# MarbleHE/ABC

Hardware: AMD Instinct MI355X
Metric: homomorphic mul+relin/sec, CKKS N=2^14 (higher is better)
Workload: dtype u64 (transforms: exact integer arithmetic in f64); 1 GPU; CKKS N=16384, 4 data limbs {50,40,40,40} + special 50-bit prime, ct x ct multiply + relinearize; total_batch=8192, batch_rank0=8192

## Files before the change

### abc_amd/csrc/abc_context.hip

```cpp
#include <cstdlib>
#include <cstring>
#include <mutex>

#include "../../include/abc_hip.h"
#include <dlfcn.h>

#include "abc_context.hpp"
#include "abc_host_math.hpp"
#include "abc_sample.hpp"

namespace abc {

static thread_local std::string g_err;
void set_error(const std::string &msg) { g_err = msg; }

static bool env_on(const char *name) {
  const char *e = std::getenv(name);
  return e && !(e[0] == '0' && e[1] == 0);
}
void read_switches(abc_hip_ctx *c) {
  abc_hip_ctx::Switches s;
  s.no_fused = env_on("ABC_HIP_NO_FUSED");
  s.no_split = env_on("ABC_HIP_NO_SPLIT");
  s.no_split4 = env_on("ABC_HIP_NO_SPLIT4");
  s.no_isplit = env_on("ABC_HIP_NO_ISPLIT");
  s.no_gsplit = env_on("ABC_HIP_NO_GSPLIT");
  s.no_bsplit = env_on("ABC_HIP_NO_BSPLIT");
  s.no_mixed = env_on("ABC_HIP_NO_MIXED");
  s.no_pack = env_on("ABC_HIP_NO_PACK");
  s.no_key_twin = env_on("ABC_HIP_NO_KEY_TWIN");
  s.no_bmul = env_on("ABC_HIP_NO_BMUL");
  s.no_iks = env_on("ABC_HIP_NO_IKS");
  s.no_lean_front = env_on("ABC_HIP_NO_LEAN_FRONT");
  s.no_tensor_intt = env_on("ABC_HIP_NO_TENSOR_INTT");
  s.no_galois_fusion = env_on("ABC_HIP_NO_GALOIS_FUSION");
  s.main_two_per_cu = env_on("ABC_HIP_MAIN_TWO_PER_CU");
  s.host_sampling = env_on("ABC_HIP_HOST_SAMPLING");
  if (const char *e = std::getenv("ABC_HIP_CHUNK")) s.chunk = (size_t)std::atol(e);
  if (const char *e = std::getenv("ABC_HIP_FEW_LIMBS")) s.few_limbs = (size_t)std::atol(e);
  if (const char *e = std::getenv("ABC_HIP_LEAN_LIMIT")) s.lean_limit = (size_t)std::atol(e);
  if (const char *e = std::getenv("ABC_HIP_PASS0_TARGET_LIMIT")) s.pass0_target_limit = (size_t)std::atol(e);
  if (const char *e = std::getenv("ABC_HIP_BFV_SCRATCH_MB")) s.bfv_scratch_mb = (size_t)std::atol(e);
  if (const char *e = std::getenv("ABC_HIP_LANES")) {
    s.lanes = std::atoi(e);
    if (s.lanes < 1) s.lanes = 1;
    if (s.lanes > abc_hip_ctx::kMaxLanes) s.lanes = abc_hip_ctx::kMaxLanes;
  }
  c->sw = s;
  RouteFacts &f = c->facts;
  f = RouteFacts{};
  f.scheme = c->scheme; f.logn = c->logn; f.K = c->K; f.L = c->L; f.nB = c->nB;
  f.use_fp = c->use_fp; f.behz_fp = c->behz_fp;
  f.big_block_log = big_block_log();
  for (int j = 0; j < c->K; j++) f.bits[j] = (unsigned char)c->h_mods[j].bits;
  f.sw = s;
  f.finish();
}

static Mod make_mod(uint64_t q, int logn, bool ntt) {
  using namespace host;
  Mod m{};
  m.q = q;
  m.two_q = 2 * q;
  const int k = bitlen(q);
  m.bits = (u32)k;
  m.shift = (u32)(k - 1);
  m.mu = (uint64_t)((((u128)1) << (k + 63)) / q);
  m.qd = (double)q;
  m.qinv = 1.0 / (double)q;
  if (ntt) {
    const uint64_t n = 1ull << logn;
    m.inv_n = invmod(n % q, q);
    m.inv_n_s = shoup(m.inv_n, q);
    if (fp_ok(m.bits)) {
      m.inv_n_c = m.inv_n > q / 2 ? -(double)(q - m.inv_n) : (double)m.inv_n;
      m.inv_n_cq = m.inv_n_c / m.qd;
    }
  }
  return m;
}

static void fill_twiddles(uint64_t q, int logn, uint64_t *dst ) {
  using namespace host;
  const size_t n = (size_t)1 << logn;
  const uint64_t psi = min_primitive_root(2 * n, q);
  uint64_t *fwd = dst, *inv = dst + 2 * n;
  uint64_t p = 1;
  for (size_t i = 0; i < n; i++) {
    fwd[2 * (size_t)bitrev((uint32_t)i, logn)] = p;
    p = mulmod(p, psi, q);
  }
  const uint64_t ipsi = invmod(psi, q);
  p = 1;
  for (size_t i = 0; i < n; i++) {
    inv[2 * (size_t)bitrev((uint32_t)i, logn)] = p;
    p = mulmod(p, ipsi, q);
  }
  for (size_t i = 0; i < n; i++) {
    fwd[2 * i + 1] = shoup(fwd[2 * i], q);
    inv[2 * i + 1] = shoup(inv[2 * i], q);
  }
}

static void fill_fp_twiddles(uint64_t q, size_t n, const uint64_t *src , double *dst ) {
  for (size_t i = 0; i < 2 * n; i++) {
    const uint64_t w = src[2 * i];
    dst[i] = w > q / 2 ? -(double)(q - w) : (double)w;
  }
}

static int build_context(abc_hip_ctx *c) {
  using namespace host;
  const int logn = c->logn, K = c->K, L = c->L;
  const size_t N = (size_t)c->n;
  const bool bfv = (c->scheme == ABC_HIP_SCHEME_BFV);
  std::vector<uint64_t> qs(c->primes.begin(), c->primes.begin() + L);
  const uint64_t qsp = c->primes[K - 1];
  DevConst &k = c->h_cst;
  std::memset(&k, 0, sizeof(k));

  c->mod_values.assign(c->primes.begin(), c->primes.end());
  std::vector<uint64_t> Bp;
  uint64_t m_sk = 0, gamma = 0;
  if (bfv) {
    bool fp_aux = !env_on("ABC_HIP_NO_FP64") && !env_on("ABC_HIP_BEHZ_SEAL_BASE");
    for (uint64_t q : c->primes) fp_aux = fp_aux && fp_ok((u32)bitlen(q));
    const int aux_bits = fp_aux ? 50 : 61;
    int nB = L;
    if (32 + bitlen(c->t) + prod_bitlen(qs) >= aux_bits * L + aux_bits) nB++;
    gamma = ntt_primes(N, 61, 2)[1];
    if (!fp_aux) {
      auto aux = ntt_primes(N, 61, (size_t)nB + 2);
      m_sk = aux[0];
      Bp.assign(aux.begin() + 2, aux.end());
    } else {
      std::vector<uint64_t> alt;
      for (uint64_t p : ntt_primes(N, 50, (size_t)nB + 1 + (size_t)K)) {
        bool clash = false;
        for (uint64_t q : c->primes) clash = clash || (p == q);
        if (!clash && alt.size() < (size_t)nB + 1) alt.push_back(p);
      }
      if (alt.size() < (size_t)nB + 1) throw std::runtime_error("not enough 50-bit NTT primes for the BEHZ auxiliary base");
      m_sk = alt[0];
      Bp.assign(alt.begin() + 1, alt.end());
    }
    c->behz_fp = fp_aux && L <= 10 && !env_on("ABC_HIP_BEHZ_INT_KERNELS");
    c->nB = nB;
    c->nBsk = nB + 1;
    for (uint64_t b : Bp) c->mod_values.push_back(b);
    c->mod_values.push_back(m_sk);
    c->mod_values.push_back(gamma);
    c->mod_values.push_back(c->t);
  }
  const int nmods = (int)c->mod_values.size();
  const int id_bsk = K, id_gamma = K + c->nBsk, id_t = K + c->nBsk + 1;
  c->h_mods.clear();
  std::vector<uint64_t> h_tw((size_t)nmods * 4 * N, 0);
  std::vector<double> h_ftw((size_t)nmods * 2 * N, 0.0);
  for (int i = 0; i < nmods; i++) {
    const bool ntt = !(bfv && i == id_gamma);
    c->h_mods.push_back(make_mod(c->mod_values[i], logn, ntt));
    if (ntt) fill_twiddles(c->mod_values[i], logn, h_tw.data() + (size_t)i * 4 * N);
    if (ntt && fp_ok(c->h_mods.back().bits))
      fill_fp_twiddles(c->mod_values[i], N, h_tw.data() + (size_t)i * 4 * N, h_ftw.data() + (size_t)i * 2 * N);
  }

  for (int j = 0; j < L; j++) {
    const uint64_t q = qs[j];
    k.inv_special[j] = invmod(qsp % q, q);
    k.inv_special_s[j] = shoup(k.inv_special[j], q);
    k.special_mod_q[j] = qsp % q;
    k.special_mod_q_s[j] = shoup(k.special_mod_q[j], q);
    k.inv_special_c[j] = k.inv_special[j] > q / 2 ? -(double)(q - k.inv_special[j]) : (double)k.inv_special[j];
    k.inv_special_cq[j] = k.inv_special_c[j] / (double)q;
    k.special_c[j] = k.special_mod_q[j] > q / 2 ? -(double)(q - k.special_mod_q[j]) : (double)k.special_mod_q[j];
    k.special_cq[j] = k.special_c[j] / (double)q;
  }
  for (int l = 1; l < L; l++)
    for (int j = 0; j < l; j++) {
      k.inv_qlast[l][j] = invmod(qs[l] % qs[j], qs[j]);
      k.inv_qlast_s[l][j] = shoup(k.inv_qlast[l][j], qs[j]);
      k.inv_qlast_c[l][j] = k.inv_qlast[l][j] > qs[j] / 2 ? -(double)(qs[j] - k.inv_qlast[l][j]) : (double)k.inv_qlast[l][j];
      k.inv_qlast_cq[l][j] = k.inv_qlast_c[l][j] / (double)qs[j];
    }

  std::vector<uint32_t> slot_map;
  if (bfv) {
    const uint64_t t = c->t;
    k.t = t;
// ... 767 lines not shown
```

### abc_amd/csrc/abc_kernels_fused.hip

```cpp
#include <type_traits>

#include "abc_context.hpp"
#include "abc_host_math.hpp"

namespace abc {

template <int LB>
__global__ __launch_bounds__((1 << LB) / 16) void k_fused_tensor_intt(DevCtx c, const u64 *__restrict__ a,
                                                                      const u64 *__restrict__ b, u64 *__restrict__ c01,
                                                                      u64 *__restrict__ c2coef, u64 *__restrict__ c2ntt, int nl) {
  __shared__ u64 lds[lds_words(LB)];
  const int j = blockIdx.x % nl;
  const size_t ct = blockIdx.x / nl;
  const size_t N = (size_t)1 << LB, pw = (size_t)nl * N;
  const Mod m = c.mods[j];
  const NttTable t = ntt_table(c, j);
  const u64 *__restrict__ a0 = a + ct * 2 * pw + j * N, *__restrict__ a1 = a0 + pw;
  const u64 *__restrict__ b0 = b + ct * 2 * pw + j * N, *__restrict__ b1 = b0 + pw;
  u64 *__restrict__ o0 = c01 + ct * 2 * pw + j * N, *__restrict__ o1 = o0 + pw;
  u64 *__restrict__ dcoef = c2coef + (ct * nl + j) * N, *__restrict__ dntt = c2ntt + (ct * nl + j) * N;
  ntt_inv_block<LB>(
      lds,
      [&](int, int i) {
        const u64 x0 = a0[i], x1 = a1[i], y0 = b0[i], y1 = b1[i];
// ... 348 lines not shown
    ntt_inv_block_a<LB, FpArith>(
        lds, ld,
        [&](int, int i, double v) {
          const double d = fp_mul_lazy(v, m.inv_n_c, m.inv_n_cq, m.qd) - (fp_from_u64(src[i]) + fix);
          o[i] = fp_to_canon(fp_mul_lazy(d, inv, inv_q, m.qd), m.qd, m.qinv);
        },
        t, m, 0, 0);
  }
}

template <int LB>
__global__ __launch_bounds__((1 << LB) / 16) void k_fused_tensor_decomp_fp(DevCtx c, const u64 *__restrict__ a,
                                                                           const u64 *__restrict__ b, u64 *__restrict__ c01,
                                                                           u64 *__restrict__ c2ntt, u64 *__restrict__ dec, int nl) {
  __shared__ double lds[lds_words(LB)];
  const int j = blockIdx.x % nl;
  const size_t ct = blockIdx.x / nl;
  const size_t N = (size_t)1 << LB;
  double src[16];
  {
    const Mod m = mod_at(c, j);
    const FpTable t = fp_table(c, j);
    TensorFront front(a, b, c01, c2ntt, ct, j, nl, N, m);
    ntt_inv_block_a<LB, FpArith>(
        lds, [&](int r, int i) { return front(r, i); },
        [&](int r, int, double v) {
          const double w = fp_centre(fp_mul_lazy(v, m.inv_n_c, m.inv_n_cq, m.qd), m.qd, m.qinv);
          src[r] = w < 0.0 ? w + m.qd : w;
        },
        t, m, 0, 0);
  }
  for (int I = 0; I <= nl; I++) {
    if (I == j) continue;
    const int ki = (I == nl) ? c.K - 1 : I;
    const Mod m = mod_at(c, ki);
    const FpTable t = fp_table(c, ki);
    u64 *__restrict__ dst = dec + ((ct * (nl + 1) + I) * nl + j) * N;
    block_sync_lds();
    ntt_fwd_block_a<LB, FpArith>(
        lds, [&](int r, int) { return src[r]; }, [&](int, int i, double v) { dst[i] = fp_to_lazy(v, m.qd, m.qinv); }, t, m, 0, 0);
  }
}

template <int LB>
__device__ __forceinline__ void store_half_done(double *__restrict__ dst, double (&y)[16], int p, const FpK &kk, int kind) {
  constexpr size_t N = (size_t)1 << LB;
  constexpr int SH = LB - 4;
  if (kind == 0) {
#pragma unroll
    for (int k = 0; k < 16; k++) dst[(k << SH) + p] = y[k];
  } else if (kind == 1) {
#pragma unroll
    for (int k = 0; k < 16; k++) pack_store<1>(dst, N, (size_t)(k << SH) + p, fp_centre(y[k], kk.q, kk.qinv));
  } else {
#pragma unroll
    for (int k = 0; k < 16; k++) pack_store<2>(dst, N, (size_t)(k << SH) + p, fp_centre(y[k], kk.q, kk.qinv));
  }
}


template <int LB, bool CKKS, bool GAL>
__global__ __launch_bounds__((1 << LB) / 16) void k_fused_operand_pass0_fp(DevCtx c, const u64 *__restrict__ src, size_t src_stride,
                                                                           double *__restrict__ part, int nl, int per_target,
                                                                           u32 gelt, int padded) {
  static_assert(LB == 14, "split transforms are laid out for N = 2^14");
  __shared__ double lds[CKKS ? lds_words(LB) : 1];
  const size_t N = (size_t)1 << LB;
  const unsigned wg = per_target ? blockIdx.x / (unsigned)(nl + 1) : blockIdx.x;
  const int only = per_target ? (int)(blockIdx.x % (unsigned)(nl + 1)) : -1;
  const int j = wg % nl;
  const size_t ct = wg / nl;
  const int tid = threadIdx.x;
  const u64 *__restrict__ sp = src + ct * src_stride + (size_t)j * N;
  double x[16];
  if constexpr (CKKS) {
    const Mod m = mod_at(c, j);
    const FpTable t = fp_table(c, j);
    ntt_inv_block_a<LB, FpArith>(
        lds, [&](int, int i) { return fp_from_u64(sp[galois_ntt_src<GAL>((u32)i, gelt, LB)]); },
        [&](int r, int, double v) {
          double w = fp_centre(fp_mul_lazy(v, m.inv_n_c, m.inv_n_cq, m.qd), m.qd, m.qinv);
          x[r] = w < 0.0 ? w + m.qd : w;
        },
        t, m, 0, 0);
  } else if (gelt) {
    const u64 qj = c.mods[j].q;
#pragma unroll
    for (int k = 0; k < 16; k++) {
      bool neg;
      const u64 v = sp[galois_coef_src((u32)((k << 10) + tid), gelt, LB, neg)];
      x[k] = fp_from_u64(neg ? neg_mod(v, qj) : v);
    }
  } else {
#pragma unroll
    for (int k = 0; k < 16; k++) x[k] = fp_from_u64(sp[(k << 10) + tid]);
  }
  const int hi0[1] = {0};
  for (int I = 0; I <= nl; I++) {
    if (CKKS && I == j) continue;
    if (only >= 0 && I != only) continue;
    const int ki = (I == nl) ? c.K - 1 : I;
    const Mod m = mod_at(c, ki);
    const FpTable t = fp_table(c, ki);
    const FpK kk = FpArith::consts(m);
    double y[16];
#pragma unroll
    for (int k = 0; k < 16; k++) y[k] = x[k];
    fwd_pass<FpArith, LB, 0, 4>(y, hi0, t, kk, 0, 0);
    double *__restrict__ dst = part + ((ct * (nl + 1) + I) * nl + j) * ((padded & 1) ? (size_t)c.ps : N);
    store_half_done<LB>(dst, y, tid, kk, ((padded & 2) && I < nl) ? pack_kind(m.bits) : 0);
  }
}

template <int LB>
__global__ __launch_bounds__((1 << LB) / 16) void k_split2_tensor_pass0_fp(DevCtx c, const u64 *__restrict__ a,
                                                                           const u64 *__restrict__ b, double *__restrict__ part,
                                                                           int nl, int pack) {
  static_assert(LB == 14, "split transforms are laid out for N = 2^14");
  __shared__ double lds[lds_words(LB)];
  const int j = blockIdx.x % nl;
  const size_t ct = blockIdx.x / nl;
  const size_t N = (size_t)1 << LB, pw = (size_t)nl * N;
  double src[16];
  {
    const Mod m = mod_at(c, j);
    const FpTable t = fp_table(c, j);
    const u64 *__restrict__ a1 = a + ct * 2 * pw + pw + (size_t)j * N, *__restrict__ b1 = b + ct * 2 * pw + pw + (size_t)j * N;
    const double q = m.qd, qinv = m.qinv;
    ntt_inv_block_a<LB, FpArith>(
        lds, [&](int, int i) { return fp_mulmod(fp_from_u64(a1[i]), fp_from_u64(b1[i]), q, qinv); },
        [&](int r, int, double v) {
          const double w = fp_centre(fp_mul_lazy(v, m.inv_n_c, m.inv_n_cq, m.qd), m.qd, m.qinv);
          src[r] = w < 0.0 ? w + m.qd : w;
        },
        t, m, 0, 0);
  }
  const int tid = threadIdx.x;
  const int hi0[1] = {0};
  for (int I = 0; I <= nl; I++) {
    if (I == j) continue;
    const int ki = (I == nl) ? c.K - 1 : I;
    const Mod m = mod_at(c, ki);
    const FpTable t = fp_table(c, ki);
    const FpK kk = FpArith::consts(m);
    double y[16];
#pragma unroll
    for (int k = 0; k < 16; k++) y[k] = src[k];
    fwd_pass<FpArith, LB, 0, 4>(y, hi0, t, kk, 0, 0);
    double *__restrict__ dst = part + ((ct * (nl + 1) + I) * nl + j) * (size_t)c.ps;
    store_half_done<LB>(dst, y, tid, kk, (pack && I < nl) ? pack_kind(m.bits) : 0);
  }
}

template <int NL>
__global__ __launch_bounds__(NL ? NL * 64 : 768) void k_split_special_fp(DevCtx c, const double *__restrict__ part, const u64 *__restrict__ key,
                                                                         const double *__restrict__ keyf, double *__restrict__ tsp_half,
                                                                         int nl_rt) {
  extern __shared__ double dyn[];
  const int nl = NL ? NL : nl_rt;
  const int J = __builtin_amdgcn_readfirstlane((int)(threadIdx.x >> 6));
  const int lane = threadIdx.x & 63;
  const int blk = blockIdx.x & 15;
  const size_t ct = (size_t)(blockIdx.x >> 4);
  const size_t N = (size_t)c.n, base = (size_t)blk << 10;
  const int ki = c.K - 1;
  const Mod m = mod_at(c, ki);
  const FpTable t = fp_table(c, ki);
  const double q = m.qd, qinv = m.qinv;
  {
    double *buf = dyn + J * lds_words(10);
    const double *__restrict__ src = part + ((ct * (nl + 1) + nl) * nl + J) * (size_t)c.ps + base;
    ntt_fwd_block_a<10, FpTail>(
        buf, [&](int, int i) { return fp_centre(src[i], q, qinv); }, [&](int, int i, double v) { buf[lds_pad(i)] = v; }, t, m, 4, blk,
        lane);
  }
  __syncthreads();
  for (int e = 2 * (int)threadIdx.x; e < 1024; e += 2 * (int)blockDim.x) {
    double s0[2] = {0.0, 0.0}, s1[2] = {0.0, 0.0};
#pragma unroll
    for (int Jx = 0; Jx < (NL ? NL : 12); Jx++) {
      if (!NL && Jx >= nl) break;
      const f64x2 v = *reinterpret_cast<const f64x2 *>(dyn + Jx * lds_words(10) + lds_pad(e));
      const size_t i0 = (((size_t)Jx * 2 + 0) * c.K + ki) * N + base + e, i1 = i0 + (size_t)c.K * N;
      f64x2 k0, k1;
      if (keyf) {
        k0 = *reinterpret_cast<const f64x2 *>(keyf + i0);
        k1 = *reinterpret_cast<const f64x2 *>(keyf + i1);
      } else {
        const u64x2 r0 = *reinterpret_cast<const u64x2 *>(key + i0), r1 = *reinterpret_cast<const u64x2 *>(key + i1);
        k0.x = fp_from_u64(r0.x); k0.y = fp_from_u64(r0.y);
        k1.x = fp_from_u64(r1.x); k1.y = fp_from_u64(r1.y);
      }
      s0[0] += fp_mulmod(v.x, k0.x, q, qinv);
      s0[1] += fp_mulmod(v.y, k0.y, q, qinv);
      s1[0] += fp_mulmod(v.x, k1.x, q, qinv);
      s1[1] += fp_mulmod(v.y, k1.y, q, qinv);
      if (Jx == 7) {
#pragma unroll
        for (int k = 0; k < 2; k++) {
          s0[k] = fp_centre(s0[k], q, qinv);
          s1[k] = fp_centre(s1[k], q, qinv);
        }
      }
    }
    f64x2 r;
    r.x = fp_centre(s0[0], q, qinv); r.y = fp_centre(s0[1], q, qinv);
    *reinterpret_cast<f64x2 *>(dyn + lds_pad(e)) = r;
    r.x = fp_centre(s1[0], q, qinv); r.y = fp_centre(s1[1], q, qinv);
    *reinterpret_cast<f64x2 *>(dyn + lds_words(10) + lds_pad(e)) = r;
  }
  __syncthreads();
  for (int comp = J; comp < 2; comp += nl) {
    double *buf = dyn + comp * lds_words(10);
    double *__restrict__ dst = tsp_half + (ct * 2 + comp) * (size_t)c.ps + base;
    ntt_inv_block_a<10, FpArith>(
        buf, [&](int, int i) { return buf[lds_pad(i)]; }, [&](int, int i, double v) { dst[i] = v; }, t, m, 4, blk, lane);
  }
}

static void launch_split_special(hipStream_t st, abc_hip_ctx *c, size_t cc, int nl, const double *part, const u64 *key, double *tsp_half) {
  const dim3 grid((unsigned)(cc * 16)), block(64 * nl);
  const size_t lds = (size_t)((nl < 2 ? 2 : nl) * lds_words(10)) * 8;
  const double *keyf = key_twin_lookup(c, key);
#define ABC_SP(NLV) hipLaunchKernelGGL((k_split_special_fp<NLV>), grid, block, lds, st, c->dc, part, key, keyf, tsp_half, nl)
  switch (nl) {
    case 1: ABC_SP(1); break;
    case 2: ABC_SP(2); break;
    case 3: ABC_SP(3); break;
    case 4: ABC_SP(4); break;
    default: ABC_SP(0); break;
  }
#undef ABC_SP
}

struct FusedScratch {
  u64 *coef, *ntt, *dec, *ksacc, *tsp, *tlast, *c01;
};
static inline FusedScratch carve(u64 *base, size_t chunk, int nl, size_t N) {
  FusedScratch s;
  s.coef = base;
  s.ntt = s.coef + chunk * nl * N;
  s.dec = s.ntt + chunk * nl * N;
  s.ksacc = s.dec + chunk * nl * (nl + 1) * N;
  s.tsp = s.ksacc + chunk * 2 * nl * N;
  s.tlast = s.tsp + chunk * 2 * N;
  s.c01 = s.tlast + chunk * 2 * N;
  return s;
}


template <int LB>
__global__ __launch_bounds__(256) void k_split3_pass_fp(DevCtx c, const double *__restrict__ tsp_half, double *__restrict__ tpart, int nl,
                                                        int pack) {
  static_assert(LB == 14, "split transforms are laid out for N = 2^14");
  const size_t cc = blockIdx.x >> 2;
  const int p = (int)((blockIdx.x & 3) << 8) + (int)threadIdx.x;
  const int hi0[1] = {0};
  double x[16];
  {
    const Mod ms = mod_at(c, c.K - 1);
    const FpTable ts = fp_table(c, c.K - 1);
    const FpK ks = FpArith::consts(ms);
    const double *__restrict__ src = tsp_half + cc * (size_t)c.ps;
#pragma unroll
    for (int k = 0; k < 16; k++) x[k] = src[(k << 10) + p];
    FpArith::centre16(x, ks);
    inv_pass<FpArith, LB, 0, 4>(x, hi0, ts, ks, 0, 0);
    const double half = (double)(ms.q >> 1);
#pragma unroll
    for (int k = 0; k < 16; k++) {
      const double w = fp_centre(fp_mul_lazy(x[k], ms.inv_n_c, ms.inv_n_cq, ms.qd) + half, ms.qd, ms.qinv);
      x[k] = w < 0.0 ? w + ms.qd : w;
    }
  }
  const u64 half = c.mods[c.K - 1].q >> 1;
  for (int j = 0; j < nl; j++) {
    const Mod m = mod_at(c, j);
    const FpTable t = fp_table(c, j);
    const FpK kk = FpArith::consts(m);
    const u64 hm = reduce64(half, m);
    const double fix = hm ? (double)(m.q - hm) : 0.0;
    double y[16];
#pragma unroll
    for (int k = 0; k < 16; k++) y[k] = x[k] + fix;
    fwd_pass<FpArith, LB, 0, 4>(y, hi0, t, kk, 0, 0);
    double *__restrict__ dst = tpart + (cc * nl + j) * (size_t)c.ps;
    store_half_done<LB>(dst, y, p, kk, pack ? pack_kind(m.bits) : 0);
  }
}

template <int MODE, bool GAL, int NL>
__global__ __launch_bounds__(NL ? (NL + 1) * 64 : 832) void k_split3_main_fp(DevCtx c, const double *__restrict__ part,
                                                                              const double *__restrict__ tpart,
                                                                              const u64 *__restrict__ opa, const u64 *__restrict__ opb,
                                                                              size_t opa_stride, size_t opb_stride, int add_c1,
                                                                              const u64 *__restrict__ key, u64 *__restrict__ out, int nl_rt,
                                                                              u32 gelt) {
  extern __shared__ double dyn[];
  const int nl = NL ? NL : nl_rt;
  const int W = __builtin_amdgcn_readfirstlane((int)(threadIdx.x >> 6));
  const int lane = threadIdx.x & 63;
  const int blk = blockIdx.x & 15;
  const int I = (int)((blockIdx.x >> 4) % nl);
  const size_t ct = (size_t)((blockIdx.x >> 4) / nl);
  const size_t N = (size_t)c.n, base = (size_t)blk << 10;
  const Mod m = mod_at(c, I);
  const FpTable t = fp_table(c, I);
  const double q = m.qd, qinv = m.qinv;
  {
    double *buf = dyn + W * lds_words(10);
    const double *__restrict__ src;
    if (W < nl - 1) {
      const int J = W < I ? W : W + 1;
      src = part + ((ct * (nl + 1) + I) * nl + J) * (size_t)c.ps + base;
    } else {
      src = tpart + ((ct * 2 + (W - (nl - 1))) * nl + I) * (size_t)c.ps + base;
    }
    ntt_fwd_block_a<10, FpArith>(
        buf, [&](int, int i) { return fp_centre(src[i], q, qinv); }, [&](int, int i, double v) { buf[lds_pad(i)] = v; }, t, m, 4, blk,
        lane);
  }
  __syncthreads();
  const double inv = c.cst->inv_special_c[I], inv_q = c.cst->inv_special_cq[I];
  const size_t pw = (size_t)nl * N;
  const double *tt0 = dyn + (nl - 1) * lds_words(10), *tt1 = dyn + nl * lds_words(10);
  for (int e = 2 * (int)threadIdx.x; e < 1024; e += 2 * (int)blockDim.x) {
    double s0[2] = {0.0, 0.0}, s1[2] = {0.0, 0.0}, d0[2] = {0.0, 0.0}, d1[2] = {0.0, 0.0};
#pragma unroll
    for (int Jx = 0; Jx < (NL ? NL : 12); Jx++) {
      if (!NL && Jx >= nl) break;
      double x[2];
      if (Jx == I) {
        if (MODE == 0) {
          const u64 *pa = opa + ct * 2 * pw + (size_t)I * N + base + e, *pb = opb + ct * 2 * pw + (size_t)I * N + base + e;
          const u64x2 a0 = *reinterpret_cast<const u64x2 *>(pa), a1 = *reinterpret_cast<const u64x2 *>(pa + pw);
          const u64x2 b0 = *reinterpret_cast<const u64x2 *>(pb), b1 = *reinterpret_cast<const u64x2 *>(pb + pw);
          const double x0[2] = {fp_from_u64(a0.x), fp_from_u64(a0.y)}, x1[2] = {fp_from_u64(a1.x), fp_from_u64(a1.y)};
          const double y0[2] = {fp_from_u64(b0.x), fp_from_u64(b0.y)}, y1[2] = {fp_from_u64(b1.x), fp_from_u64(b1.y)};
#pragma unroll
          for (int k = 0; k < 2; k++) {
            x[k] = fp_mulmod(x1[k], y1[k], q, qinv);
            d0[k] = fp_mulmod(x0[k], y0[k], q, qinv);
            d1[k] = fp_mulmod(x0[k], y1[k], q, qinv) + fp_mulmod(x1[k], y0[k], q, qinv);
          }
        } else {
          const u64 *xl = opa + ct * opa_stride + (size_t)I * N;
#pragma unroll
          for (int k = 0; k < 2; k++) {
            const u32 si = galois_ntt_src<GAL>((u32)(base + e + k), gelt, c.logn);
            x[k] = fp_from_u64(xl[si]);
            if (opb) {
              const u64 *ad = opb + ct * opb_stride + (size_t)I * N;
              d0[k] = fp_from_u64(ad[si]);
              if (add_c1) d1[k] = fp_from_u64(ad[pw + si]);
            }
          }
        }
      } else {
        const int w = Jx < I ? Jx : Jx - 1;
        const f64x2 v = *reinterpret_cast<const f64x2 *>(dyn + w * lds_words(10) + lds_pad(e));
        x[0] = v.x;
        x[1] = v.y;
      }
      const u64x2 k0 = *reinterpret_cast<const u64x2 *>(key + (((size_t)Jx * 2 + 0) * c.K + I) * N + base + e);
      const u64x2 k1 = *reinterpret_cast<const u64x2 *>(key + (((size_t)Jx * 2 + 1) * c.K + I) * N + base + e);
      s0[0] += fp_mulmod(x[0], fp_from_u64(k0.x), q, qinv);
      s0[1] += fp_mulmod(x[1], fp_from_u64(k0.y), q, qinv);
      s1[0] += fp_mulmod(x[0], fp_from_u64(k1.x), q, qinv);
      s1[1] += fp_mulmod(x[1], fp_from_u64(k1.y), q, qinv);
      if (Jx == 7) {
#pragma unroll
        for (int k = 0; k < 2; k++) {
          s0[k] = fp_centre(s0[k], q, qinv);
          s1[k] = fp_centre(s1[k], q, qinv);
        }
      }
    }
    const f64x2 u0 = *reinterpret_cast<const f64x2 *>(tt0 + lds_pad(e)), u1 = *reinterpret_cast<const f64x2 *>(tt1 + lds_pad(e));
    u64x2 r;
    r.x = fp_to_canon(fp_mul_lazy(s0[0] - u0.x, inv, inv_q, q) + d0[0], q, qinv);
    r.y = fp_to_canon(fp_mul_lazy(s0[1] - u0.y, inv, inv_q, q) + d0[1], q, qinv);
    *reinterpret_cast<u64x2 *>(out + ((ct * 2 + 0) * nl + I) * N + base + e) = r;
    r.x = fp_to_canon(fp_mul_lazy(s1[0] - u1.x, inv, inv_q, q) + d1[0], q, qinv);
// ... 482 lines not shown
```

### abc_amd/csrc/abc_ntt.hpp

```cpp
#pragma once

#include "abc_modarith.hpp"

namespace abc {

__device__ __forceinline__ int lds_pad(int i) { return i + ((i >> 6) << 2); }
constexpr int lds_words(int lb) { return (1 << lb) + ((1 << lb) >> 6) * 4; }

struct NttTable {
  const u64x2 *tw;
  const u64x2 *itw;
};
struct alignas(16) f64x2 {
  double x, y;
};
#define ABC_CONST_AS __attribute__((address_space(4)))
struct FpTable {
  const ABC_CONST_AS double *tw, *itw;
};
__device__ __forceinline__ double tw_load(const ABC_CONST_AS double *p) { return *p; }
__device__ __forceinline__ u64x2 tw_load(const u64x2 *p) { return *p; }

struct FpK {
  double q, qinv;
// ... 389 lines not shown
    else fwd_pass<A, LB, S, R>(x, hi, t, kk, S0, b);
    if constexpr (SC::R3 == 0) {
#pragma unroll
      for (int g = 0; g < P::NG; g++)
#pragma unroll
        for (int k = 0; k < (1 << R); k++) store(g * (1 << R) + k, P::elem(hi[g], lo[g], k), x[g * (1 << R) + k]);
      return;
    } else {
      lds_store<LB, S, R>(lds, x, hi, lo);
    }
  }
  if constexpr (SC::R3 != 0) {
    wave_sync();
    constexpr int S = SC::R0 + SC::R1 + SC::R2, R = SC::R3;
    using P = PassIdx<LB, S, R>;
    int hi[P::NG], lo[P::NG];
    P::groups(tid, hi, lo);
    lds_load<LB, S, R>(lds, x, hi, lo);
    A::template fwd_begin<3>(x, kk);
    if constexpr (LTW && !P::UNIFORM) fwd_pass_lds<A, LB, S, R>(x, hi, ltw, kk);
    else fwd_pass<A, LB, S, R>(x, hi, t, kk, S0, b);
#pragma unroll
    for (int g = 0; g < P::NG; g++)
#pragma unroll
      for (int k = 0; k < (1 << R); k++) store(g * (1 << R) + k, P::elem(hi[g], lo[g], k), x[g * (1 << R) + k]);
  }
}


template <class A, class Store>
__device__ __forceinline__ void ntt_fwd_tail1024_pairs(typename A::E *lds, typename A::E (&x)[16], Store store,
                                                       const typename A::Table &t, const Mod &m, int S0, int b, int lane,
                                                       const typename A::TW *ltw) {
  constexpr int LB = 10;
  const typename A::K kk = A::consts(m);
  {
    const int hi[2] = {0, 0};
    fwd_pass<A, LB, 0, 3>(x, hi, t, kk, S0, b);
#pragma unroll
    for (int k = 0; k < 8; k++) {
      typename A::E *p = lds + lds_pad((k << 7) + 2 * lane);
      p[0] = x[k];
      p[1] = x[8 + k];
    }
  }
  wave_sync();
  {
    using P = PassIdx<LB, 3, 4>;
    int hi[P::NG], lo[P::NG];
    P::groups(lane, hi, lo);
    lds_load<LB, 3, 4>(lds, x, hi, lo);
    A::template fwd_begin<1>(x, kk);
    fwd_pass_lds<A, LB, 3, 4>(x, hi, ltw, kk);
    lds_store<LB, 3, 4>(lds, x, hi, lo);
  }
  wave_sync();
  {
    using P = PassIdx<LB, 7, 3>;
    int hi[P::NG], lo[P::NG];
    P::groups(lane, hi, lo);
    lds_load<LB, 7, 3>(lds, x, hi, lo);
    A::template fwd_begin<2>(x, kk);
    fwd_pass_lds<A, LB, 7, 3>(x, hi, ltw, kk);
#pragma unroll
    for (int g = 0; g < P::NG; g++)
#pragma unroll
      for (int k = 0; k < 8; k++) store(g * 8 + k, P::elem(hi[g], lo[g], k), x[g * 8 + k]);
  }
}

template <int LB, bool GUARD = true, class Load, class Store>
__device__ __forceinline__ void ntt_fwd_block(u64 *lds, Load load, Store store, const NttTable &t, const Mod &m, int S0,
                                              int b) {
  ntt_fwd_block_a<LB, IntArith<GUARD>>(lds, load, store, t, m, S0, b);
}

template <int LB, class A, class Load, class Store, bool LTW = false>
__device__ __forceinline__ void ntt_inv_block_a(typename A::E *lds, Load load, Store store, const typename A::Table &t,
                                                const Mod &m, int S0, int b, int tid_in = -1,
                                                const typename A::TW *ltw = nullptr ) {
  using SC = Sched<LB>;
  const int tid = tid_in < 0 ? (int)threadIdx.x : tid_in;
  const typename A::K kk = A::consts(m);
  typename A::E x[16];
  constexpr int SA = SC::R0, SB = SC::R0 + SC::R1, SCc = SC::R0 + SC::R1 + SC::R2;
  if constexpr (SC::R3 != 0) {
    constexpr int S = SCc, R = SC::R3;
    using P = PassIdx<LB, S, R>;
    int hi[P::NG], lo[P::NG];
    P::groups(tid, hi, lo);
#pragma unroll
    for (int g = 0; g < P::NG; g++)
#pragma unroll
      for (int k = 0; k < (1 << R); k++) x[g * (1 << R) + k] = load(g * (1 << R) + k, P::elem(hi[g], lo[g], k));
    A::template inv_begin<0>(x, kk);
    if constexpr (LTW && !P::UNIFORM) inv_pass_lds<A, LB, S, R>(x, hi, ltw, kk);
    else inv_pass<A, LB, S, R>(x, hi, t, kk, S0, b);
    lds_store<LB, S, R>(lds, x, hi, lo);
    wave_sync();
  }
  {
    constexpr int S = SB, R = SC::R2;
    using P = PassIdx<LB, S, R>;
    int hi[P::NG], lo[P::NG];
    P::groups(tid, hi, lo);
    if constexpr (SC::R3 != 0) {
      lds_load<LB, S, R>(lds, x, hi, lo);
    } else {
#pragma unroll
      for (int g = 0; g < P::NG; g++)
#pragma unroll
        for (int k = 0; k < (1 << R); k++) x[g * (1 << R) + k] = load(g * (1 << R) + k, P::elem(hi[g], lo[g], k));
    }
    A::template inv_begin<(SC::R3 != 0 ? 1 : 0)>(x, kk);
    if constexpr (LTW && !P::UNIFORM) inv_pass_lds<A, LB, S, R>(x, hi, ltw, kk);
    else inv_pass<A, LB, S, R>(x, hi, t, kk, S0, b);
    lds_store<LB, S, R>(lds, x, hi, lo);
    wave_sync();
  }
  {
    constexpr int S = SA, R = SC::R1;
    using P = PassIdx<LB, S, R>;
    int hi[P::NG], lo[P::NG];
    P::groups(tid, hi, lo);
    lds_load<LB, S, R>(lds, x, hi, lo);
    A::template inv_begin<(SC::R3 != 0 ? 2 : 1)>(x, kk);
    if constexpr (LTW && !P::UNIFORM) inv_pass_lds<A, LB, S, R>(x, hi, ltw, kk);
    else inv_pass<A, LB, S, R>(x, hi, t, kk, S0, b);
    lds_store<LB, S, R>(lds, x, hi, lo);
    if constexpr (LB <= 10) wave_sync(); else block_sync_lds();
  }
  {
    constexpr int S = 0, R = SC::R0;
    using P = PassIdx<LB, S, R>;
    int hi[P::NG], lo[P::NG];
    P::groups(tid, hi, lo);
    lds_load<LB, S, R>(lds, x, hi, lo);
    A::template inv_begin<(SC::R3 != 0 ? 3 : 2)>(x, kk);
    if constexpr (LTW && !P::UNIFORM) inv_pass_lds<A, LB, S, R>(x, hi, ltw, kk);
    else inv_pass<A, LB, S, R>(x, hi, t, kk, S0, b);
#pragma unroll
    for (int g = 0; g < P::NG; g++)
#pragma unroll
      for (int k = 0; k < (1 << R); k++) store(g * (1 << R) + k, P::elem(hi[g], lo[g], k), x[g * (1 << R) + k]);
  }
}

template <int LB, class Load, class Store>
__device__ __forceinline__ void ntt_inv_block(u64 *lds, Load load, Store store, const NttTable &t, const Mod &m, int S0,
                                              int b) {
  ntt_inv_block_a<LB, IntArith<true>>(lds, load, store, t, m, S0, b);
}

__device__ __forceinline__ u64 canon4(u64 v, const Mod &m) { return csub(csub(v, m.two_q), m.q); }
__device__ __forceinline__ u64 canon32(u64 v, const Mod &m) {
  v = csub(v, m.two_q << 4);
  v = csub(v, m.two_q << 3);
  v = csub(v, m.two_q << 2);
  v = csub(v, m.two_q << 1);
  return canon4(v, m);
}
template <bool GUARD>
__device__ __forceinline__ u64 canon_fwd(u64 v, const Mod &m) { return GUARD ? canon4(v, m) : canon32(v, m); }
__host__ __device__ __forceinline__ bool unguarded_ok(u32 bits) { return bits <= 57; }
__device__ __forceinline__ u64 scale_inv_n(u64 v, const Mod &m) { return mul_shoup(v, m.inv_n, m.inv_n_s, m.q); }

}
```

### abc_amd/csrc/abc_route.hpp

```cpp
#pragma once

#include <cstddef>
#include <cstdint>
#include <cstdio>

namespace abc {

struct Switches {
  bool no_fused = false, no_split = false, no_split4 = false, no_isplit = false, no_gsplit = false, no_lean_front = false, no_bsplit = false, no_mixed = false, no_pack = false, no_key_twin = false, no_bmul = false, no_iks = false, no_tensor_intt = false;
  bool no_galois_fusion = false;
  bool main_two_per_cu = false;
  bool host_sampling = false;
  size_t chunk = 0, few_limbs = 48, lean_limit = 96, bfv_scratch_mb = 0, pass0_target_limit = 128;
  int lanes = 2;
};

constexpr unsigned kFpBits = 50;
constexpr unsigned kLazyBits = 55;
constexpr unsigned kUnguardedBits = 57;
constexpr unsigned kIsplitBits = 60;

constexpr size_t fused_scratch_limbs(int nl) { return (size_t)nl * (nl + 1) + 6 * (size_t)nl + 4; }

struct RouteFacts {
  int scheme = 0, logn = 0, K = 0, L = 0, nB = 0;
  bool use_fp = true, behz_fp = false;
  int big_block_log = 12;
  unsigned char bits[17] = {};
  Switches sw;
  unsigned widest = 0;
  uint32_t fp_mask = 0;
  bool all_fp = false;
  bool guard = false;
  bool lazy = false;
  void finish() {
    widest = 0;
    fp_mask = 0;
    for (int j = 0; j < K; j++) {
      if (bits[j] > widest) widest = bits[j];
      if (bits[j] <= kFpBits) fp_mask |= 1u << j;
    }
    all_fp = use_fp && widest <= kFpBits;
    guard = widest > kUnguardedBits;
    lazy = widest <= kLazyBits;
  }
  uint32_t fp_data_mask(int nl) const { return fp_mask & ((1u << nl) - 1u); }
  bool data_fp(int nl) const { return fp_data_mask(nl) == (1u << nl) - 1u; }
  bool special_fp() const { return K > 0 && ((fp_mask >> (K - 1)) & 1u); }
};

enum class Seq {
  split14,
  gsplit15,
  isplit,
  bsplit14,
  bsplit_big,
  lds_fp,
  lds_int,
  bmul,
  generic
};
enum class KsFront { plain, fp, iks };
enum class BfvMul { behz, split, big };
enum class Rescale { generic, fp, mixed };

struct KsRoute {
  Seq seq;
  KsFront front;
};
struct MulRoute {
  Seq seq;
  BfvMul mul;
  KsRoute ks;
};
struct RotRoute {
  bool fold;
  KsRoute ks;
};
struct RescaleRoute {
  Rescale kind;
  uint32_t fpmask;
};

namespace route_detail {
inline bool gsplit_ok(const RouteFacts &f, int nl) {
  return f.logn == 15 && f.scheme == 2 && f.use_fp && !f.sw.no_gsplit && nl >= 1 && nl <= 15 && f.widest <= kFpBits;
}
inline bool bsplit_ok(const RouteFacts &f, int nl) {
  return f.logn == 14 && f.scheme == 1 && f.use_fp && !f.sw.no_bsplit && nl >= 1 && nl <= 8 && f.widest <= kFpBits;
}
inline bool bsplit_big_ok(const RouteFacts &f, int nl) {
  return (f.logn == 13 || f.logn == 15 || f.logn == 16) && f.scheme == 1 && f.use_fp && !f.sw.no_bsplit && !f.sw.no_gsplit && nl >= 1 &&
         nl <= 8 && f.widest <= kFpBits;
}
inline bool isplit_ok(const RouteFacts &f, int nl) {
  if ((f.logn != 14 && f.logn != 15) || f.scheme != 2 || f.sw.no_fused || f.sw.no_split || f.sw.no_isplit || nl < 1 ||
      nl > (f.logn == 15 ? 15 : 7))
    return false;
  if (f.logn == 15 && f.sw.no_gsplit) return false;
  return f.widest <= kIsplitBits;
}
inline bool bmul_shape(const RouteFacts &f, int limbs) {
  return f.scheme == 1 && f.use_fp && f.behz_fp && !f.sw.no_bmul && !f.sw.no_split && !f.sw.no_fused && f.L == limbs && f.nB == limbs &&
         f.K == f.L + 1;
}
inline bool bmul_relin_ok(const RouteFacts &f) {
  if (f.logn == 13) return bmul_shape(f, 4) && bsplit_big_ok(f, f.L);
  return f.logn == 14 && bmul_shape(f, 8) && bsplit_ok(f, f.L);
}
inline Seq lds_seq(const RouteFacts &f, int nl, bool mul) {
  const bool ckks = f.scheme == 2;
  if (f.logn == 14 && ckks && !f.all_fp && isplit_ok(f, nl)) return Seq::isplit;
  if (f.logn == 14 && ckks && f.all_fp && !f.sw.no_split && nl <= 12) return Seq::split14;
  if (!mul && f.logn == 14 && !ckks && !f.sw.no_split && bsplit_ok(f, nl)) return Seq::bsplit14;
  return f.all_fp ? Seq::lds_fp : Seq::lds_int;
}
}

inline KsFront route_ks_front(const RouteFacts &f, int nl) {
  if (f.logn > 14 && f.use_fp && f.data_fp(nl) && f.special_fp()) return KsFront::fp;
  if ((f.logn == 15 || f.logn == 16) && !f.sw.no_iks && f.big_block_log == 12) return KsFront::iks;
  return KsFront::plain;
}

inline KsRoute route_keyswitch(const RouteFacts &f, int nl) {
  using namespace route_detail;
  const KsRoute generic{Seq::generic, route_ks_front(f, nl)};
  if (f.logn == 15 && gsplit_ok(f, nl)) return {Seq::gsplit15, KsFront::plain};
  if (f.logn == 15 && f.scheme == 2 && !f.all_fp && isplit_ok(f, nl)) return {Seq::isplit, KsFront::plain};
  if (bsplit_big_ok(f, nl)) return {Seq::bsplit_big, KsFront::plain};
  if (f.logn > 14 || f.logn < 10 || f.sw.no_fused) return generic;
  return {lds_seq(f, nl, false), KsFront::plain};
}

inline BfvMul route_bfv_multiply(const RouteFacts &f) {
  using namespace route_detail;
  if (f.logn == 14) return bmul_relin_ok(f) ? BfvMul::split : BfvMul::behz;
  if (f.logn == 13) return bmul_shape(f, 4) ? BfvMul::big : BfvMul::behz;
  return ((f.logn == 15 || f.logn == 16) && bmul_shape(f, 8) && !f.sw.no_gsplit && f.big_block_log == 12) ? BfvMul::big : BfvMul::behz;
}

inline MulRoute route_mul_relin(const RouteFacts &f, int nl) {
  using namespace route_detail;
  const KsRoute none{Seq::generic, KsFront::plain};
  if (f.scheme == 2) {
    if (f.logn == 15 && gsplit_ok(f, nl)) return {Seq::gsplit15, BfvMul::behz, none};
    if (f.logn == 15 && !f.all_fp && isplit_ok(f, nl)) return {Seq::isplit, BfvMul::behz, none};
    if (f.logn <= 14 && f.logn >= 10 && !f.sw.no_fused) return {lds_seq(f, nl, true), BfvMul::behz, none};
    return {Seq::generic, BfvMul::behz, route_keyswitch(f, nl)};
  }
  if (bmul_relin_ok(f)) return {Seq::bmul, BfvMul::split, none};
  return {Seq::generic, route_bfv_multiply(f), route_keyswitch(f, nl)};
}

inline RotRoute route_rotate(const RouteFacts &f, int nl, bool in_place) {
  using namespace route_detail;
  const bool may_fold = !in_place && !f.sw.no_galois_fusion;
  if (may_fold && f.logn == 15 && gsplit_ok(f, nl)) return {true, {Seq::gsplit15, KsFront::plain}};
  if (may_fold && f.logn == 15 && f.scheme == 2 && !f.all_fp && isplit_ok(f, nl)) return {true, {Seq::isplit, KsFront::plain}};
  if (may_fold && f.scheme == 1) {
    if (!f.sw.no_split && !f.sw.no_fused) {
      if (f.logn == 14 && bsplit_ok(f, nl)) return {true, {Seq::bsplit14, KsFront::plain}};
      if (bsplit_big_ok(f, nl)) return {true, {Seq::bsplit_big, KsFront::plain}};
    }
// ... 114 lines not shown
```

Before: 436,100 mul+relin/s.

## Prefetch special-prime key words during forward NTT and split inverse NTT across wavefronts

For four data limbs, the special-prime key-switch kernel now issues its key loads into registers before and after the forward NTT, so global-memory latency overlaps with NTT compute. The per-element inner product then reads those preloaded values. The two inverse NTTs, which previously ran on only two of the four wavefronts, are split so that each pair of wavefronts does half of one 1024-point transform, with inverse twiddles loaded early. The cost is higher register pressure from the prefetched key array, and an env switch restores the serial path.

After: 437,600 mul+relin/s (median of 3 runs). About the same (+0.3%).

```diff
diff --git a/abc_amd/csrc/abc_context.hip b/abc_amd/csrc/abc_context.hip
--- a/abc_amd/csrc/abc_context.hip
+++ b/abc_amd/csrc/abc_context.hip
@@ -35,6 +35,7 @@
   s.no_tensor_intt = env_on("ABC_HIP_NO_TENSOR_INTT");
   s.no_galois_fusion = env_on("ABC_HIP_NO_GALOIS_FUSION");
   s.main_two_per_cu = env_on("ABC_HIP_MAIN_TWO_PER_CU");
+  s.special_serial = env_on("ABC_HIP_SPECIAL_SERIAL");
   s.host_sampling = env_on("ABC_HIP_HOST_SAMPLING");
   if (const char *e = std::getenv("ABC_HIP_CHUNK")) s.chunk = (size_t)std::atol(e);
   if (const char *e = std::getenv("ABC_HIP_FEW_LIMBS")) s.few_limbs = (size_t)std::atol(e);
diff --git a/abc_amd/csrc/abc_kernels_fused.hip b/abc_amd/csrc/abc_kernels_fused.hip
--- a/abc_amd/csrc/abc_kernels_fused.hip
+++ b/abc_amd/csrc/abc_kernels_fused.hip
@@ -524,10 +524,39 @@
   }
 }
 
-template <int NL>
+#ifndef ABC_HIP_SPECIAL_HALVES
+#define ABC_HIP_SPECIAL_HALVES 1
+#endif
+#ifndef ABC_HIP_SPECIAL_TWIDDLES_AHEAD
+#define ABC_HIP_SPECIAL_TWIDDLES_AHEAD 1
+#endif
+constexpr bool kSpecialHalves = ABC_HIP_SPECIAL_HALVES, kSpecialTwiddlesAhead = ABC_HIP_SPECIAL_TWIDDLES_AHEAD;
+__device__ __forceinline__ void special_pair_products(double (&s0)[2], double (&s1)[2], const f64x2 v, const f64x2 k0, const f64x2 k1,
+                                                      int Jx, double q, double qinv) {
+  s0[0] += fp_mulmod(v.x, k0.x, q, qinv);
+  s0[1] += fp_mulmod(v.y, k0.y, q, qinv);
+  s1[0] += fp_mulmod(v.x, k1.x, q, qinv);
+  s1[1] += fp_mulmod(v.y, k1.y, q, qinv);
+  if (Jx == 7) {
+#pragma unroll
+    for (int k = 0; k < 2; k++) {
+      s0[k] = fp_centre(s0[k], q, qinv);
+      s1[k] = fp_centre(s1[k], q, qinv);
+    }
+  }
+}
+__device__ __forceinline__ void special_park(double *dyn, int e, const double (&s0)[2], const double (&s1)[2], double q, double qinv) {
+  f64x2 r;
+  r.x = fp_centre(s0[0], q, qinv); r.y = fp_centre(s0[1], q, qinv);
+  *reinterpret_cast<f64x2 *>(dyn + lds_pad(e)) = r;
+  r.x = fp_centre(s1[0], q, qinv); r.y = fp_centre(s1[1], q, qinv);
+  *reinterpret_cast<f64x2 *>(dyn + lds_words(10) + lds_pad(e)) = r;
+}
+template <int NL, bool SERIAL>
 __global__ __launch_bounds__(NL ? NL * 64 : 768) void k_split_special_fp(DevCtx c, const double *__restrict__ part, const u64 *__restrict__ key,
                                                                          const double *__restrict__ keyf, double *__restrict__ tsp_half,
                                                                          int nl_rt) {
+  static_assert(NL == 4 || SERIAL, "the form with loads ahead is laid out for four wavefronts");
   extern __shared__ double dyn[];
   const int nl = NL ? NL : nl_rt;
   const int J = __builtin_amdgcn_readfirstlane((int)(threadIdx.x >> 6));
@@ -539,54 +568,103 @@
   const Mod m = mod_at(c, ki);
   const FpTable t = fp_table(c, ki);
   const double q = m.qd, qinv = m.qinv;
+  constexpr int W = NL ? 2 * NL : 1;
+  u64x2 kw[2][W];
+  auto request = [&](int r, u64x2 (&w)[W]) {
+    const size_t at = base + 2 * threadIdx.x + r * 512;
+#pragma unroll
+    for (int Jc = 0; Jc < 2 * NL; Jc++) {
+      const size_t i = ((size_t)Jc * c.K + ki) * N + at;
+      if (keyf) {
+        const f64x2 d = *reinterpret_cast<const f64x2 *>(keyf + i);
+        w[Jc].x = (u64)__double_as_longlong(d.x);
+        w[Jc].y = (u64)__double_as_longlong(d.y);
+      } else {
+        w[Jc] = *reinterpret_cast<const u64x2 *>(key + i);
+      }
+    }
+  };
+  auto pair_trip = [&](auto twin, int r, const u64x2 (&w)[W]) {
+    const int e = 2 * (int)threadIdx.x + r * 512;
+    auto key_pair = [&](const u64x2 &kwd) {
+      f64x2 k;
+      if (decltype(twin)::value) {
+        k.x = __longlong_as_double((long long)kwd.x); k.y = __longlong_as_double((long long)kwd.y);
+      } else {
+        k.x = fp_from_u64(kwd.x); k.y = fp_from_u64(kwd.y);
+      }
+      return k;
+    };
+    double s0[2] = {0.0, 0.0}, s1[2] = {0.0, 0.0};
+#pragma unroll
+    for (int Jx = 0; Jx < NL; Jx++) {
+      const f64x2 v = *reinterpret_cast<const f64x2 *>(dyn + Jx * lds_words(10) + lds_pad(e));
+      special_pair_products(s0, s1, v, key_pair(w[2 * Jx]), key_pair(w[2 * Jx + 1]), Jx, q, qinv);
+    }
+    special_park(dyn, e, s0, s1, q, qinv);
+  };
   {
     double *buf = dyn + J * lds_words(10);
     const double *__restrict__ src = part + ((ct * (nl + 1) + nl) * nl + J) * (size_t)c.ps + base;
+    if constexpr (!SERIAL) request(0, kw[0]);
     ntt_fwd_block_a<10, FpTail>(
         buf, [&](int, int i) { return fp_centre(src[i], q, qinv); }, [&](int, int i, double v) { buf[lds_pad(i)] = v; }, t, m, 4, blk,
         lane);
+    if constexpr (!SERIAL) request(1, kw[1]);
   }
   __syncthreads();
-  for (int e = 2 * (int)threadIdx.x; e < 1024; e += 2 * (int)blockDim.x) {
-    double s0[2] = {0.0, 0.0}, s1[2] = {0.0, 0.0};
-#pragma unroll
-    for (int Jx = 0; Jx < (NL ? NL : 12); Jx++) {
-      if (!NL && Jx >= nl) break;
-      const f64x2 v = *reinterpret_cast<const f64x2 *>(dyn + Jx * lds_words(10) + lds_pad(e));
-      const size_t i0 = (((size_t)Jx * 2 + 0) * c.K + ki) * N + base + e, i1 = i0 + (size_t)c.K * N;
-      f64x2 k0, k1;
-      if (keyf) {
-        k0 = *reinterpret_cast<const f64x2 *>(keyf + i0);
-        k1 = *reinterpret_cast<const f64x2 *>(keyf + i1);
-      } else {
-        const u64x2 r0 = *reinterpret_cast<const u64x2 *>(key + i0), r1 = *reinterpret_cast<const u64x2 *>(key + i1);
-        k0.x = fp_from_u64(r0.x); k0.y = fp_from_u64(r0.y);
-        k1.x = fp_from_u64(r1.x); k1.y = fp_from_u64(r1.y);
-      }
-      s0[0] += fp_mulmod(v.x, k0.x, q, qinv);
-      s0[1] += fp_mulmod(v.y, k0.y, q, qinv);
-      s1[0] += fp_mulmod(v.x, k1.x, q, qinv);
-      s1[1] += fp_mulmod(v.y, k1.y, q, qinv);
-      if (Jx == 7) {
-#pragma unroll
-        for (int k = 0; k < 2; k++) {
-          s0[k] = fp_centre(s0[k], q, qinv);
-          s1[k] = fp_centre(s1[k], q, qinv);
+  constexpr bool HALVES = !SERIAL && kSpecialHalves;
+  double wa[7], wb[7];
+  auto inverse_twiddles = [&]() {
+    const int p = ((J & 1) << 6) + lane;
+    half_inv_twiddles<FpArith, 7>(t, 4, blk, p, wa);
+    half_inv_twiddles<FpArith, 4>(t, 4, blk, p >> 3, wb);
+  };
+  if constexpr (SERIAL) {
+    for (int e = 2 * (int)threadIdx.x; e < 1024; e += 2 * (int)blockDim.x) {
+      double s0[2] = {0.0, 0.0}, s1[2] = {0.0, 0.0};
+#pragma unroll
+      for (int Jx = 0; Jx < (NL ? NL : 12); Jx++) {
+        if (!NL && Jx >= nl) break;
+        const f64x2 v = *reinterpret_cast<const f64x2 *>(dyn + Jx * lds_words(10) + lds_pad(e));
+        const size_t i0 = (((size_t)Jx * 2 + 0) * c.K + ki) * N + base + e, i1 = i0 + (size_t)c.K * N;
+        f64x2 k0, k1;
+        if (keyf) {
+          k0 = *reinterpret_cast<const f64x2 *>(keyf + i0);
+          k1 = *reinterpret_cast<const f64x2 *>(keyf + i1);
+        } else {
+          const u64x2 r0 = *reinterpret_cast<const u64x2 *>(key + i0), r1 = *reinterpret_cast<const u64x2 *>(key + i1);
+          k0.x = fp_from_u64(r0.x); k0.y = fp_from_u64(r0.y);
+          k1.x = fp_from_u64(r1.x); k1.y = fp_from_u64(r1.y);
         }
-      }
-    }
-    f64x2 r;
-    r.x = fp_centre(s0[0], q, qinv); r.y = fp_centre(s0[1], q, qinv);
-    *reinterpret_cast<f64x2 *>(dyn + lds_pad(e)) = r;
-    r.x = fp_centre(s1[0], q, qinv); r.y = fp_centre(s1[1], q, qinv);
-    *reinterpret_cast<f64x2 *>(dyn + lds_words(10) + lds_pad(e)) = r;
+        special_pair_products(s0, s1, v, k0, k1, Jx, q, qinv);
+      }
+      special_park(dyn, e, s0, s1, q, qinv);
+    }
+  } else {
+#pragma unroll
+    for (int r = 0; r < 2; r++) {
+      if (keyf) pair_trip(std::true_type{}, r, kw[r]);
+      else pair_trip(std::false_type{}, r, kw[r]);
+      if constexpr (HALVES && kSpecialTwiddlesAhead) {
+        if (r == 0) inverse_twiddles();
+      }
+    }
   }
   __syncthreads();
-  for (int comp = J; comp < 2; comp += nl) {
-    double *buf = dyn + comp * lds_words(10);
+  if constexpr (HALVES) {
+    if constexpr (!kSpecialTwiddlesAhead) inverse_twiddles();
+    const int comp = J >> 1;
     double *__restrict__ dst = tsp_half + (ct * 2 + comp) * (size_t)c.ps + base;
-    ntt_inv_block_a<10, FpArith>(
-        buf, [&](int, int i) { return buf[lds_pad(i)]; }, [&](int, int i, double v) { dst[i] = v; }, t, m, 4, blk, lane);
+    ntt_inv_half1024_a<FpArith>(
+        dyn + comp * lds_words(10), [&](int i, double v) { dst[i] = v; }, t, m, 4, blk, J & 1, lane, wa, wb);
+  } else {
+    for (int comp = J; comp < 2; comp += nl) {
+      double *buf = dyn + comp * lds_words(10);
+      double *__restrict__ dst = tsp_half + (ct * 2 + comp) * (size_t)c.ps + base;
+      ntt_inv_block_a<10, FpArith>(
+          buf, [&](int, int i) { return buf[lds_pad(i)]; }, [&](int, int i, double v) { dst[i] = v; }, t, m, 4, blk, lane);
+    }
   }
 }
 
@@ -594,13 +672,17 @@
   const dim3 grid((unsigned)(cc * 16)), block(64 * nl);
   const size_t lds = (size_t)((nl < 2 ? 2 : nl) * lds_words(10)) * 8;
   const double *keyf = key_twin_lookup(c, key);
-#define ABC_SP(NLV) hipLaunchKernelGGL((k_split_special_fp<NLV>), grid, block, lds, st, c->dc, part, key, keyf, tsp_half, nl)
+  const bool serial = c->sw.special_serial;
+#define ABC_SP(NLV, SER) hipLaunchKernelGGL((k_split_special_fp<NLV, SER>), grid, block, lds, st, c->dc, part, key, keyf, tsp_half, nl)
   switch (nl) {
-    case 1: ABC_SP(1); break;
-    case 2: ABC_SP(2); break;
-    case 3: ABC_SP(3); break;
-    case 4: ABC_SP(4); break;
-    default: ABC_SP(0); break;
+    case 1: ABC_SP(1, true); break;
+    case 2: ABC_SP(2, true); break;
+    case 3: ABC_SP(3, true); break;
+    case 4:
+      if (serial) ABC_SP(4, true);
+      else ABC_SP(4, false);
+      break;
+    default: ABC_SP(0, true); break;
   }
 #undef ABC_SP
 }
diff --git a/abc_amd/csrc/abc_ntt.hpp b/abc_amd/csrc/abc_ntt.hpp
--- a/abc_amd/csrc/abc_ntt.hpp
+++ b/abc_amd/csrc/abc_ntt.hpp
@@ -565,6 +565,81 @@
   ntt_inv_block_a<LB, IntArith<true>>(lds, load, store, t, m, S0, b);
 }
 
+struct HalfInvSched { static constexpr int RA = 3, RB = 3, RC = 3, RX = 1; };
+template <class A, int S>
+__device__ __forceinline__ void half_inv_twiddles(const typename A::Table &t, int S0, int b, int hi, typename A::TW (&w)[7]) {
+#pragma unroll
+  for (int u = 0; u < 3; u++)
+#pragma unroll
+    for (int j = 0; j < (1 << u); j++) w[(1 << u) - 1 + j] = tw_load(t.itw + (1 << (S0 + S + u)) + (b << (S + u)) + (hi << u) + j);
+}
+template <class A>
+__device__ __forceinline__ void inv_pass8(typename A::E (&x)[8], const typename A::TW (&w)[7], const typename A::K &kk) {
+#pragma unroll
+  for (int u = 2; u >= 0; u--) {
+    const int half = 1 << (2 - u);
+#pragma unroll
+    for (int k = 0; k < 8; k++) {
+      if (k & half) continue;
+      A::inv(x[k], x[k | half], w[(1 << u) - 1 + (k >> (3 - u))], kk);
+    }
+  }
+}
+template <class A, class Store>
+__device__ __forceinline__ void ntt_inv_half1024_a(typename A::E *lds, Store store, const typename A::Table &t, const Mod &m,
+                                                   int S0, int b, int h, int lane, const typename A::TW (&wa)[7],
+                                                   const typename A::TW (&wb)[7]) {
+  using HS = HalfInvSched;
+  static_assert(HS::RA == 3 && HS::RB == 3 && HS::RC == 3 && HS::RX == 1, "eight values per lane: three radix-8 passes and one stage");
+  constexpr int SA = HS::RX + HS::RC + HS::RB, SB = HS::RX + HS::RC, SCc = HS::RX;
+  const typename A::K kk = A::consts(m);
+  const int p = (h << 6) + lane;
+  typename A::E x[8];
+  {
+    typename A::E *e = lds + lds_pad(p << (10 - SA));
+#pragma unroll
+    for (int k = 0; k < 8; k++) x[k] = e[k];
+    inv_pass8<A>(x, wa, kk);
+#pragma unroll
+    for (int k = 0; k < 8; k++) e[k] = x[k];
+  }
+  wave_sync();
+  {
+    const int at = ((p >> 3) << (10 - SB)) + (p & 7);
+#pragma unroll
+    for (int k = 0; k < 8; k++) x[k] = fp_centre(lds[lds_pad(at + (k << 3))], kk.q, kk.qinv);
+    inv_pass8<A>(x, wb, kk);
+#pragma unroll
+    for (int k = 0; k < 8; k++) lds[lds_pad(at + (k << 3))] = x[k];
+  }
+  wave_sync();
+  const int at = (h << (10 - SCc)) + lane;
+  {
+    typename A::TW wc[7];
+    half_inv_twiddles<A, SCc>(t, S0, b, h, wc);
+#pragma unroll
+    for (int k = 0; k < 8; k++) x[k] = fp_centre(lds[lds_pad(at + (k << 6))], kk.q, kk.qinv);
+    inv_pass8<A>(x, wc, kk);
+  }
+  typename A::E mine[4];
+#pragma unroll
+  for (int j = 0; j < 4; j++) {
+    mine[j] = h ? x[4 + j] : x[j];
+    lds[lds_pad(at + ((h ? j : 4 + j) << 6))] = h ? x[j] : x[4 + j];
+  }
+  block_sync_lds();
+  const typename A::TW w0 = tw_load(t.itw + (1 << S0) + b);
+#pragma unroll
+  for (int j = 0; j < 4; j++) {
+    const int i = ((4 * h + j) << 6) + lane;
+    const typename A::E other = lds[lds_pad(i + (h ? 0 : 512))];
+    typename A::E X = h ? other : mine[j], Y = h ? mine[j] : other;
+    A::inv(X, Y, w0, kk);
+    store(i, X);
+    store(i + 512, Y);
+  }
+}
+
 __device__ __forceinline__ u64 canon4(u64 v, const Mod &m) { return csub(csub(v, m.two_q), m.q); }
 __device__ __forceinline__ u64 canon32(u64 v, const Mod &m) {
   v = csub(v, m.two_q << 4);
diff --git a/abc_amd/csrc/abc_route.hpp b/abc_amd/csrc/abc_route.hpp
--- a/abc_amd/csrc/abc_route.hpp
+++ b/abc_amd/csrc/abc_route.hpp
@@ -10,6 +10,7 @@
   bool no_fused = false, no_split = false, no_split4 = false, no_isplit = false, no_gsplit = false, no_lean_front = false, no_bsplit = false, no_mixed = false, no_pack = false, no_key_twin = false, no_bmul = false, no_iks = false, no_tensor_intt = false;
   bool no_galois_fusion = false;
   bool main_two_per_cu = false;
+  bool special_serial = false;
   bool host_sampling = false;
   size_t chunk = 0, few_limbs = 48, lean_limit = 96, bfv_scratch_mb = 0, pass0_target_limit = 128;
   int lanes = 2;
```
